# qwertyhgb/Prostate-Cancer-Multimodal-Segmentation

Hardware: AMD Instinct MI355X
Metric: train volumes/sec (5ch 128x128x64) (higher is better)
Workload: dtype bf16; 1 GPU; UNet3D 5->1, 2 x 5x128x128x64 per GPU, BCEDiceLoss, Adam(1e-4, wd 1e-5); global_batch=2, parallelism=dp1

## Files before the change

include/pcms_hip.h:

```cpp
#ifndef PCMS_HIP_H
#define PCMS_HIP_H
#include <hip/hip_runtime.h>

#ifdef __cplusplus
extern "C" {
#endif

#define PCMS_CONV_ACCUMULATE 1
#define PCMS_CONV_RELU 2
#define PCMS_GRAD_STORE 1
#define PCMS_STEM_DENSE 16

int pcms_pack_input(int dtype, const float* in, void* out, int N, int Cin, long V, int Cp, hipStream_t s);

int pcms_conv3_chunk(int dtype);
int pcms_conv3_pack_elems(int dtype, int J, int Kdim);
int pcms_conv3_mblocks(int N, int D, int H, int W);
int pcms_conv3_fwd_rows(int dtype, int N, int D, int H, int W, int c0, int c1, int Cout);
int pcms_conv3_big_min_boxes(int v);
int pcms_conv3_big_max_wgs(int v);
int pcms_conv3_small_box_mtw2(int v);
int pcms_conv3_fwd_box_vol(int v);
int pcms_conv3_pack(int dtype, const float* w, void* out, int Cout, int Cin, int flip, hipStream_t s);
int pcms_conv3_pack2(int dtype, const float* w, void* fwd, void* dgrad, int Cout, int Cin, hipStream_t s);
// ... 68 lines not shown
int pcms_bn_relu_bwd(int dtype, const void* da, const void* y, const float* scale, const float* shift,
                     const float* mean, const float* invstd, const float* gamma, float* part, float* coef,
                     float* dgamma, float* dbeta, void* dy, int C, long nvox, double* ws, hipStream_t s);
int pcms_bn_relu_bwd_finish(int dtype, const void* da, const void* y, const float* scale, const float* shift,
                            const float* mean, const float* invstd, const float* gamma, const float* part,
                            int rows, float* coef, float* dgamma, float* dbeta, void* dy, int C, long nvox,
                            double* ws, hipStream_t s);

int pcms_maxpool_fwd(int dtype, const void* a, void* p, int N, int D, int H, int W, int C, hipStream_t s);
int pcms_maxpool_bwd(int dtype, const void* a, const void* dp, void* da, int N, int D, int H, int W,
                     int C, hipStream_t s);
int pcms_bn_relu_pool(int dtype, const void* y, void* a, void* p, const float* scale, const float* shift,
                      int N, int D, int H, int W, int C, hipStream_t s);
int pcms_maxpool_bwd_bn_rows(int dtype, int N, int D, int H, int W, int C);
int pcms_maxpool_bwd_bn(int dtype, const void* y, const float* scale, const float* shift, const float* mean,
                        const float* invstd, const void* dp, void* da, float* part, int N, int D, int H, int W,
                        int C, hipStream_t s);
int pcms_maxpool_bwd_bn_sums(int dtype, const void* y, const float* scale, const float* shift, const float* mean,
                             const float* invstd, const void* dp, const void* da, float* part, int N, int D, int H,
                             int W, int C, hipStream_t s);
int pcms_maxpool_bn_apply(int dtype, const void* y, const float* scale, const float* shift, const float* mean,
                          const float* invstd, const float* coef, const void* dp, const void* da, void* dy, int N,
                          int D, int H, int W, int C, hipStream_t s);

int pcms_convt_fwd_stream(int v);
int pcms_convt_pack_elems(int dtype, int Cin, int Cout);
int pcms_convt_pack(int dtype, const float* w, void* out, int Cin, int Cout, int dgrad, hipStream_t s);
int pcms_convt_fwd(int dtype, const void* x, const void* wpack, const float* bias, void* out,
                   int N, int Din, int Hin, int Win, int Cin, int Cout, int Do, int Ho, int Wo, hipStream_t s);
int pcms_convt_fwd_ws_floats(int N, int Din, int Hin, int Win, int Cin, int Cout);
int pcms_convt_fwd_ws(int dtype, const void* x, const void* wpack, const float* bias, void* out, float* ws,
                      int N, int Din, int Hin, int Win, int Cin, int Cout, int Do, int Ho, int Wo, hipStream_t s);
int pcms_convt_dgrad(int dtype, const void* dout, const void* wpack_d, void* dx,
                     int N, int Din, int Hin, int Win, int Cin, int Cout, int Do, int Ho, int Wo, hipStream_t s);
int pcms_convt_dgrad_ws_floats(int N, int Din, int Hin, int Win, int Cin, int Cout);
int pcms_convt_dgrad_ws(int dtype, const void* dout, const void* wpack_d, void* dx, float* ws,
                        int N, int Din, int Hin, int Win, int Cin, int Cout, int Do, int Ho, int Wo, hipStream_t s);
int pcms_convt_wgrad_ws_floats(int N, int Din, int Hin, int Win, int Cin, int Cout, int target_wgs);
int pcms_convt_reduce_fused(int v);
int pcms_convt_wgrad_taps(int tt);
int pcms_convt_wgrad(int dtype, const void* x, const void* dout, float* dw, float* ws,
                     int N, int Din, int Hin, int Win, int Cin, int Cout, int Do, int Ho, int Wo,
                     int target_wgs, hipStream_t s);
int pcms_convt_wgrad_bias_ws_floats(int dtype, int N, int Din, int Hin, int Win, int Cin, int Cout, int target_wgs);
int pcms_convt_wgrad_bias(int dtype, const void* x, const void* dout, float* dw, float* db, float* ws, float* bws,
                          int N, int Din, int Hin, int Win, int Cin, int Cout, int Do, int Ho, int Wo,
// ... 131 lines not shown
```

prostate-cancer-multimodal-segmentation_amd/_lib.py:

```python
from __future__ import annotations

import ctypes
import os

import torch

LIB_PATH = os.environ.get("PCMS_LIB") or os.path.join(os.path.dirname(os.path.abspath(__file__)), "libpcms_hip.so")

F32, BF16, F32X3 = 0, 1, 2

SIGNATURES = {
    "pcms_pack_input": "ippiilis",
    "pcms_conv3_chunk": "i",
    "pcms_conv3_pack_elems": "iii",
    "pcms_conv3_mblocks": "iiii",
    "pcms_conv3_fwd_rows": "iiiiiiii",
    "pcms_conv3_big_min_boxes": "i",
    "pcms_conv3_big_max_wgs": "i",
    "pcms_conv3_fwd_box_vol": "i",
    "pcms_conv3_small_box_mtw2": "i",
    "pcms_conv3_pack": "ippiiis",
    "pcms_conv3_pack2": "ipppiis",
    "pcms_conv3_splits": "iii",
    "pcms_conv3_fwd": "ipipippppippiiiiiiis",
# ... 24 lines not shown
    "pcms_stem_wgrad": "ppppiiiiis",
    "pcms_stem_wgrad_bn": "ppppppppppiiiiis",
    "pcms_stem_dgrad_pack_elems": "i",
    "pcms_stem_dgrad_pack": "ippis",
    "pcms_stem_dgrad": "ipppiiiiis",
    "pcms_bn_relu_bwd_eval": "ipppppils",
    "pcms_head_bn_bwd_eval": "ippppppliis",
    "pcms_split_epilogue_rows": "l",
    "pcms_split_epilogue": "ipipppipilis",
    "pcms_bn_ws_doubles": "i",
    "pcms_bn_finalize": "piidpppppffppppps",
    "pcms_bn_eval_coeffs": "ppppfipps",
    "pcms_bn_fold": "ppppppfilpps",
    "pcms_bn_relu": "ippppils",
    "pcms_bn_bwd_rows": "iil",
    "pcms_bn_relu_bwd": "i" + "p" * 12 + "ilps",
    "pcms_maxpool_fwd": "ippiiiiis",
    "pcms_maxpool_bwd": "ipppiiiiis",
    "pcms_bn_relu_pool": "ipppppiiiiis",
    "pcms_maxpool_bwd_bn_rows": "iiiiii",
    "pcms_maxpool_bwd_bn": "ippppppppiiiiis",
    "pcms_maxpool_bwd_bn_sums": "ippppppppiiiiis",
    "pcms_maxpool_bn_apply": "ipppppppppiiiiis",
    "pcms_bn_relu_bwd_finish": "i" + "p" * 8 + "ippppilps",
    "pcms_convt_pack": "ippiiis",
    "pcms_convt_pack_elems": "iii",
    "pcms_convt_fwd_stream": "i",
    "pcms_convt_fwd": "ippppiiiiiiiiis",
    "pcms_convt_fwd_ws_floats": "iiiiii",
    "pcms_convt_fwd_ws": "ipppppiiiiiiiiis",
    "pcms_convt_dgrad": "ipppiiiiiiiiis",
    "pcms_convt_dgrad_ws_floats": "iiiiii",
    "pcms_convt_dgrad_ws": "ippppiiiiiiiiis",
    "pcms_convt_wgrad_ws_floats": "iiiiiii",
    "pcms_convt_wgrad_taps": "i",
    "pcms_convt_reduce_fused": "i",
    "pcms_bn_bwd_rows_cap": "i",
    "pcms_stream_grid_cap": "i",
    "pcms_convt_wgrad": "ippppiiiiiiiiiis",
    "pcms_convt_wgrad_bias_ws_floats": "iiiiiiii",
    "pcms_convt_wgrad_bias": "ippppppiiiiiiiiiis",
    "pcms_box_channel_sum_ws_floats": "iiiiii",
    "pcms_box_channel_sum": "ipppiiiiiiiiiiis",
    "pcms_head_fwd": "ippppliiifs",
    "pcms_head_bwd_ws_floats": "lii",
    "pcms_head_bwd": "ipppppppliis",
# ... 127 lines not shown
```

prostate-cancer-multimodal-segmentation_amd/csrc/ops_pool.hip:

```cpp
#include "ops_units.h"
#include "pcms_hip.h"

namespace {

template <typename T>
__global__ void maxpool_fwd_kernel(const T* a, T* p, int N, int D, int H, int W, int C) {
  constexpr int VEC = Elem<T>::kVec;
  const int Do = D / 2, Ho = H / 2, Wo = W / 2, CV = C / VEC;
  const long total = (long)N * Do * Ho * Wo * CV;
  for (long i = blockIdx.x * (long)blockDim.x + threadIdx.x; i < total; i += (long)gridDim.x * blockDim.x) {
    const uint32_t ii = (uint32_t)i;
    const int cv = ii % CV; uint32_t r = ii / CV;
    const int wo = r % Wo; r /= Wo;
    const int ho = r % Ho; r /= Ho;
    const int d_o = r % Do; const long n = r / Do;
    float m[VEC];
#pragma unroll
    for (int j = 0; j < VEC; ++j) m[j] = -INFINITY;
    for (int k = 0; k < 8; ++k) {
      const long vin = ((n * D + 2 * d_o + (k >> 2)) * H + 2 * ho + ((k >> 1) & 1)) * W + 2 * wo + (k & 1);
      float v[VEC];
      load16<T>(a + vin * C + cv * VEC, v);
#pragma unroll
      for (int j = 0; j < VEC; ++j)
// ... 19 lines not shown
#pragma unroll
    for (int j = 0; j < VEC; ++j) { m[j] = -INFINITY; arg[j] = 0; }
    long vin[8];
    for (int k = 0; k < 8; ++k) {
      vin[k] = ((n * D + 2 * d_o + (k >> 2)) * H + 2 * ho + ((k >> 1) & 1)) * W + 2 * wo + (k & 1);
      float v[VEC];
      load16<T>(a + vin[k] * C + cv * VEC, v);
#pragma unroll
      for (int j = 0; j < VEC; ++j)
        if (v[j] > m[j] || (v[j] != v[j] && m[j] == m[j])) { m[j] = v[j]; arg[j] = k; }
    }
    float g[VEC];
    load16<T>(dp + i * VEC, g);
    for (int k = 0; k < 8; ++k) {
      float o[VEC];
      load16<T>(da + vin[k] * C + cv * VEC, o);
#pragma unroll
      for (int j = 0; j < VEC; ++j) o[j] += (arg[j] == k) ? g[j] : 0.f;
      store16<T>(da + vin[k] * C + cv * VEC, o);
    }
  }
}

template <typename T, bool NT>
__global__ void __launch_bounds__(TPB) bn_relu_pool_kernel(const T* y, T* a, T* p, const float* scale,
                                                           const float* shift, int N, int D, int H, int W,
                                                           int C) {
  constexpr int VEC = Elem<T>::kVec;
  const int Dc = (D + 1) / 2, Hc = (H + 1) / 2, Wc = (W + 1) / 2, CV = C / VEC;
  const int Do = D / 2, Ho = H / 2, Wo = W / 2;
  const long total = (long)N * Dc * Hc * Wc * CV;
  const long stride = (long)gridDim.x * blockDim.x;
  long i = blockIdx.x * (long)blockDim.x + threadIdx.x;
  const int cv = (int)(i % CV);
  float sc[VEC], sh[VEC];
#pragma unroll
  for (int j = 0; j < VEC; ++j) { sc[j] = scale[cv * VEC + j]; sh[j] = shift[cv * VEC + j]; }
  for (; i < total; i += stride) {
    uint32_t r = (uint32_t)(i / CV);
    const int wc = r % Wc; r /= Wc;
    const int hc = r % Hc; r /= Hc;
    const int dc = r % Dc; const long n = r / Dc;
    float m[VEC];
#pragma unroll
    for (int j = 0; j < VEC; ++j) m[j] = -INFINITY;
    float v[8][VEC];
    long vin[8];
    bool in[8];
#pragma unroll
    for (int k = 0; k < 8; ++k) {
      const int d = 2 * dc + (k >> 2), h = 2 * hc + ((k >> 1) & 1), w = 2 * wc + (k & 1);
      in[k] = d < D && h < H && w < W;
      vin[k] = ((n * D + d) * H + h) * W + w;
#ifndef BRP_NTLOAD
#define BRP_NTLOAD 1
#endif
      if (in[k]) ld16<NT && BRP_NTLOAD>(y + vin[k] * C + cv * VEC, v[k]);
    }
#pragma unroll
    for (int k = 0; k < 8; ++k) {
      if (!in[k]) continue;
#pragma unroll
      for (int j = 0; j < VEC; ++j) v[k][j] = round_st<T>(bn_relu1(v[k][j], sc[j], sh[j]));
      st16<NT>(a + vin[k] * C + cv * VEC, v[k]);
#pragma unroll
      for (int j = 0; j < VEC; ++j)
        if (v[k][j] > m[j] || v[k][j] != v[k][j]) m[j] = v[k][j];
    }
    if (dc < Do && hc < Ho && wc < Wo) store16<T>(p + (((n * Do + dc) * Ho + hc) * Wo + wc) * C + cv * VEC, m);
  }
}

template <typename T, bool STORE = true>
__global__ void __launch_bounds__(TPB, 3) maxpool_bwd_bn_kernel(const T* y, const float* scale, const float* shift,
                                                             const float* mean, const float* invstd, const T* dp,
                                                             T* da, float* part, int N, int D, int H, int W,
                                                             int C) {
  constexpr int VEC = Elem<T>::kVec;
  __shared__ float red[TPB][VEC][2];
  const int Dc = (D + 1) / 2, Hc = (H + 1) / 2, Wc = (W + 1) / 2, CV = C / VEC;
  const int Do = D / 2, Ho = H / 2, Wo = W / 2;
  const long total = (long)N * Dc * Hc * Wc * CV;
  const long stride = (long)gridDim.x * blockDim.x;
  long i = blockIdx.x * (long)blockDim.x + threadIdx.x;
  const int cv = (int)(i % CV);
  float sc[VEC], sh[VEC], mu[VEC], is[VEC], sg[VEC], sgx[VEC];
#pragma unroll
  for (int j = 0; j < VEC; ++j) {
    const int c = cv * VEC + j;
    sc[j] = scale[c]; sh[j] = shift[c]; mu[j] = mean[c]; is[j] = invstd[c];
    sg[j] = 0.f; sgx[j] = 0.f;
  }
  auto unpack = [](const u32x4_t r, float (&o)[VEC]) {
    if constexpr (sizeof(T) == 2) {
#pragma unroll
      for (int q = 0; q < 4; ++q) { o[2 * q] = __uint_as_float(r[q] << 16); o[2 * q + 1] = __uint_as_float(r[q] & 0xffff0000u); }
    } else {
#pragma unroll
      for (int q = 0; q < 4; ++q) o[q] = __uint_as_float(r[q]);
    }
  };
  for (; i < total; i += stride) {
    uint32_t r = (uint32_t)(i / CV);
    const int wc = r % Wc; r /= Wc;
    const int hc = r % Hc; r /= Hc;
    const int dc = r % Dc; const long n = r / Dc;
    const bool whole = dc < Do && hc < Ho && wc < Wo;
    u32x4_t yr[8], dr[8], gr = {0u, 0u, 0u, 0u};
    const long v0 = ((n * D + 2 * dc) * H + 2 * hc) * W + 2 * wc;
    const bool ind = 2 * dc + 1 < D, inh = 2 * hc + 1 < H, inw = 2 * wc + 1 < W;
    auto vk = [&](int k) { return v0 + (long)(k >> 2) * H * W + ((k >> 1) & 1) * W + (k & 1); };
    auto ink = [&](int k) { return (!(k & 4) || ind) && (!(k & 2) || inh) && (!(k & 1) || inw); };
#pragma unroll
    for (int k = 0; k < 8; ++k) {
      yr[k] = (u32x4_t){0u, 0u, 0u, 0u};
      dr[k] = yr[k];
      if (ink(k)) {
        yr[k] = *reinterpret_cast<const u32x4_t*>(y + vk(k) * C + cv * VEC);
        dr[k] = *reinterpret_cast<const u32x4_t*>(da + vk(k) * C + cv * VEC);
      }
    }
    if (whole) gr = *reinterpret_cast<const u32x4_t*>(dp + (((n * Do + dc) * Ho + hc) * Wo + wc) * C + cv * VEC);
    float g[VEC], m[VEC];
    int arg[VEC];
    unpack(gr, g);
#pragma unroll
    for (int j = 0; j < VEC; ++j) { m[j] = -INFINITY; arg[j] = 0; }
    auto round2 = [](f32x2_t v) -> f32x2_t {
      if constexpr (sizeof(T) == 2) {
        const uint32_t u = pack_bf16x2(v[0], v[1]);
        return (f32x2_t){__uint_as_float(u << 16), __uint_as_float(u & 0xffff0000u)};
      } else {
        return v;
      }
    };
    auto z2of = [&](const float (&yv)[VEC], int q) {
      return __builtin_elementwise_fma((f32x2_t){yv[2 * q], yv[2 * q + 1]}, (f32x2_t){sc[2 * q], sc[2 * q + 1]},
                                       (f32x2_t){sh[2 * q], sh[2 * q + 1]});
    };
    if (whole) {
#pragma unroll
      for (int k = 0; k < 8; ++k) {
        float yv[VEC];
        unpack(yr[k], yv);
#pragma unroll
        for (int j = 0; j < VEC; ++j) {
          const float av = round_st<T>(bn_relu1(yv[j], sc[j], sh[j]));
          if (av > m[j] || (av != av && m[j] == m[j])) { m[j] = av; arg[j] = k; }
        }
      }
    }
#pragma unroll
    for (int k = 0; k < 8; ++k) {
      if (!ink(k)) continue;
      float yv[VEC], o[VEC];
      u32x4_t yk = yr[k];
      asm volatile("" : "+v"(yk));
      unpack(yk, yv);
      unpack(dr[k], o);
      if (whole) {
#pragma unroll
        for (int j = 0; j < VEC; ++j) o[j] += (arg[j] == k) ? g[j] : 0.f;
        if constexpr (STORE) store16<T>(da + vk(k) * C + cv * VEC, o);
// ... 98 lines not shown
          if (av > m[j] || (av != av && m[j] == m[j])) { m[j] = av; arg[j] = k; }
        }
      }
    }
#pragma unroll
    for (int k = 0; k < 8; ++k) {
      if (!ink(k)) continue;
      float yv[VEC], o[VEC], out[VEC];
      u32x4_t yk = yr[k];
      asm volatile("" : "+v"(yk));
      unpack(yk, yv);
      unpack(dr[k], o);
      if (whole) {
#pragma unroll
        for (int j = 0; j < VEC; ++j) o[j] = round_st<T>(o[j] + ((arg[j] == k) ? g[j] : 0.f));
      }
#pragma unroll
      for (int j = 0; j < VEC; ++j) out[j] = bn_bwd_dy(o[j], yv[j], sc[j], sh[j], mu[j], is[j], k1[j], k2[j], k3[j]);
      st16<NT>(dy + vk(k) * C + cv * VEC, out);
    }
  }
}

}

static int cell_grid(long total, int CV, int cap) {
  int g = stream_grid(total, TPB, cap);
  const int per = CV / std::__gcd(CV, TPB);
  return std::max(per, g / per * per);
}
static int pool_cells(int N, int D, int H, int W, long* cells) {
  *cells = (long)N * ((D + 1) / 2) * ((H + 1) / 2) * ((W + 1) / 2);
  return *cells * 8 >= (1L << 31) ? -7 : 0;
}
static bool pool_nt(int dtype, int N, int D, int H, int W, int C) {
  return (long)N * D * H * W * C * bytes_of(dtype) >= kNtBytesBn;
}

extern "C" {

int pcms_maxpool_fwd(int dtype, const void* a, void* p, int N, int D, int H, int W, int C, hipStream_t s) {
  if ((long)N * D * H * W * C >= (1L << 31)) return -7;
  const long total = (long)N * (D / 2) * (H / 2) * (W / 2) * (C / vec_of(dtype));
  const int grid = stream_grid(total, TPB);
  return for_storage(dtype, [&](auto t) {
    using T = decltype(t);
// ... 5 lines not shown
int pcms_maxpool_bwd(int dtype, const void* a, const void* dp, void* da, int N, int D, int H, int W, int C,
                     hipStream_t s) {
  if ((long)N * D * H * W * C >= (1L << 31)) return -7;
  const long total = (long)N * (D / 2) * (H / 2) * (W / 2) * (C / vec_of(dtype));
  const int grid = stream_grid(total, TPB);
  return for_storage(dtype, [&](auto t) {
    using T = decltype(t);
    hipLaunchKernelGGL(maxpool_bwd_kernel<T>, dim3(grid), dim3(TPB), 0, s, (const T*)a, (const T*)dp, (T*)da, N, D, H,
                       W, C);
    PCMS_CHECK_LAUNCH();
  });
}

int pcms_bn_relu_pool(int dtype, const void* y, void* a, void* p, const float* scale, const float* shift, int N,
                      int D, int H, int W, int C, hipStream_t s) {
  const int VEC = vec_of(dtype), CV = C / VEC;
  if (C % VEC) return -1;
  long cells;
  if (const int rc = pool_cells(N, D, H, W, &cells)) return rc;
  const int grid = cell_grid(cells * CV, CV, 8192);
  return for_stream(dtype, pool_nt(dtype, N, D, H, W, C), [&](auto t, auto nt) {
    using T = decltype(t);
    hipLaunchKernelGGL((bn_relu_pool_kernel<T, decltype(nt)::value>), dim3(grid), dim3(TPB), 0, s, (const T*)y, (T*)a,
                       (T*)p, scale, shift, N, D, H, W, C);
    PCMS_CHECK_LAUNCH();
  });
}

int pcms_maxpool_bwd_bn_rows(int dtype, int N, int D, int H, int W, int C) {
  const int CV = C / vec_of(dtype);
  long cells;
  pool_cells(N, D, H, W, &cells);
  return cell_grid(cells * CV, CV, g_bn_rows_cap);
}

static int maxpool_bwd_bn_any(bool store, int dtype, const void* y, const float* scale, const float* shift,
                              const float* mean, const float* invstd, const void* dp, void* da, float* part, int N,
                              int D, int H, int W, int C, hipStream_t s) {
  const int VEC = vec_of(dtype);
  if (C % VEC || TPB % (C / VEC)) return -1;
  long cells;
  if (const int rc = pool_cells(N, D, H, W, &cells)) return rc;
  const int grid = pcms_maxpool_bwd_bn_rows(dtype, N, D, H, W, C);
  return for_stream(dtype, store, [&](auto t, auto st) {
    using T = decltype(t);
    hipLaunchKernelGGL((maxpool_bwd_bn_kernel<T, decltype(st)::value>), dim3(grid), dim3(TPB), 0, s, (const T*)y, scale,
                       shift, mean, invstd, (const T*)dp, (T*)da, part, N, D, H, W, C);
    PCMS_CHECK_LAUNCH();
  });
}

int pcms_maxpool_bwd_bn(int dtype, const void* y, const float* scale, const float* shift, const float* mean,
                        const float* invstd, const void* dp, void* da, float* part, int N, int D, int H, int W,
                        int C, hipStream_t s) {
  return maxpool_bwd_bn_any(true, dtype, y, scale, shift, mean, invstd, dp, da, part, N, D, H, W, C, s);
}

int pcms_maxpool_bwd_bn_sums(int dtype, const void* y, const float* scale, const float* shift, const float* mean,
                             const float* invstd, const void* dp, const void* da, float* part, int N, int D, int H,
                             int W, int C, hipStream_t s) {
  return maxpool_bwd_bn_any(false, dtype, y, scale, shift, mean, invstd, dp, const_cast<void*>(da), part, N, D, H, W,
                            C, s);
}

int pcms_maxpool_bn_apply(int dtype, const void* y, const float* scale, const float* shift, const float* mean,
                          const float* invstd, const float* coef, const void* dp, const void* da, void* dy, int N,
                          int D, int H, int W, int C, hipStream_t s) {
  const int VEC = vec_of(dtype), CV = C / VEC;
  if (C % VEC || TPB % CV) return -1;
  long cells;
// ... 12 lines not shown
```

prostate-cancer-multimodal-segmentation_amd/engine.py:

```python
from __future__ import annotations

import contextlib
import math
import os
from typing import Dict, List, NamedTuple, Optional, Tuple

import torch

from . import _lib
from ._lib import BF16, F32, F32X3, call, query
from .dp import module_grad_ranges
from .packs import BN_EPS, WeightPacks, gaps

BN_MOMENTUM = 0.1

_DT = {"bf16": (torch.bfloat16, BF16), "fp32": (torch.float32, F32)}


class Route(NamedTuple):
    kind: str
    splits: int
    slabs: int
    slabs16: int
    rows: int
    pack16: bool


class Layout(NamedTuple):
    N: int
    D: int
    H: int
    W: int
    act_ckpt: bool
    side_min_level: int
    convt_wgrad_side: bool
    pool_bn_apply_fused: bool
    wgrad_target: int
    split_target: int
    fuse_bnin: bool
    use_b16: bool
    switches: Tuple[int, ...]
    fwd: Tuple[Route, ...] = ()
    dgrad: Tuple[Optional[Route], ...] = ()
    bnin: Tuple[bool, ...] = ()
    pool_rows: Tuple[int, ...] = ()


class ConvSpec:
    __slots__ = ("mod", "cin", "cout", "cin_store", "fwd", "dgrad", "code", "fwd16", "dgrad16", "i")

    def __init__(self, mod, cin, cout, cin_store):
        self.mod, self.cin, self.cout, self.cin_store = mod, cin, cout, cin_store
        self.i = None
        self.fwd = None
        self.dgrad = None
        self.fwd16 = None
        self.dgrad16 = None
        self.code = None

# ... 56 lines not shown
            cs.code, cs.i = self.code, i
        self.stem_fast = self.code == BF16 and self.cp == 8
        self.stem_sup = 0
        self.stem_dense = 16 if self.nmod <= 5 else 0
        self.fuse_bnin = True
        self.use_b16 = os.environ.get("PCMS_B16", "1") != "0"
        self.packs = WeightPacks(self)
        self._flat_ptrs = None
        self.bufs = None
        self.buf_key = None
        self.layout: Optional[Layout] = None
        self.epoch = 0
        self.saved_epoch = -1
        self.saved_eval_epoch = -1
        self._folded = False
        self.act_ckpt = False
        self.split_target = 512
        self.wgrad_target = 256
        self.grad_ready = None
        self.kernel_timer = None
        self.wgrad_side_min_level = 99
        self.convt_wgrad_side = False
        self.pool_bn_apply_fused = False
        self._side_stream = None
        self._side_used = False
        self.fold_bn_eval = True
        self._bn_epoch = 0
        self._store_ranges = None
        self._gstore = False
        self._flatten()
        for bn in self.bns:
            c = bn.c
            bn.scale, bn.shift, bn.mean, bn.invstd = (torch.empty(c, device=device) for _ in range(4))

    def set_fp32_conv_mode(self, mode: str, convs=None):
        if self.code == BF16:
            raise ValueError("the bf16 build has one conv arithmetic")
        code = {"x6": F32, "x3": F32X3}[mode]
        changed = [cs for cs in self.convs if convs is None or cs.i in convs]
        for cs in changed:
            cs.code = code
        self.packs.recoded(changed)
        self.buf_key = None

    def _flatten(self):
        params = list(self.model.parameters())
# ... 188 lines not shown
            rows = query("pcms_split_epilogue_rows", N * S[0] * S[1] * S[2])
        return Route(kind, splits, slabs, sp16, rows, pack16)

    def _alloc(self, key):
        L = Layout(*key)
        N, D, H, W = key[:4]
        self.bufs = self.layout = self.buf_key = None
        S = self._levels(D, H, W)
        if min(S[4]) < 1:
            raise ValueError(f"spatial size {(D, H, W)} is too small for 4 poolings")
        nv = [N * d * h * w for (d, h, w) in S]
        C = [64 * (1 << l) for l in range(5)]
        T = self.tdtype
        dev = self.device

        def act(l, c):
            return torch.empty(nv[l] * c, dtype=T, device=dev)

        b: Dict[str, object] = {"S": S, "nv": nv, "C": C}
        b["xin"] = act(0, self.cp)
        for l in range(5):
            if l > 0:
                b[f"pool{l}"] = act(l, C[l - 1])
            for k in ("y1", "a1", "y2", "x"):
                b[f"e{l}_{k}"] = act(l, C[l])
        for l in range(4):
            for k in (("u", "a2") if L.act_ckpt else ("u", "y1", "a1", "y2", "a2")):
                b[f"d{l}_{k}"] = act(l, C[l]) if (l, k) != (0, "a2") else None
        if L.act_ckpt:
            for k in ("y1", "a1", "y2"):
                b[f"ck_{k}"] = act(0, C[0])
        for l in range(5):
            b[f"gx{l}"] = act(l, C[l])
            b[f"gA{l}"] = act(l, C[l])
            b[f"gY{l}"] = act(l, C[l])
            b[f"gZ{l}"] = act(l, C[l]) if l >= L.side_min_level else b[f"gY{l}"]
            b[f"gU{l}"] = act(l, C[l])
        self.stem_sup = query("pcms_stem_supported", N, D, H, W) if self.stem_fast else 0
        b16 = L.use_b16 and self.code == BF16
        bnin = tuple(self._bnin(blk, N, S[l]) for blk, l in zip(self.enc + self.dec, (0, 1, 2, 3, 4, 3, 2, 1, 0)))
        rows_f = max(max(query("pcms_conv3_mblocks", N, *S[l]) for l in range(5)),
                     query("pcms_stem_fwd_rows", N, *S[0]))
        ws = [query("pcms_stem_wgrad_ws_floats", N, *S[0], self.nmod)] if self.stem_fast else [1]
        yacc = 1
        fwd, dgrad = [], []
        for cs, l, c0, c1 in self._sites():
# ... 79 lines not shown

    def _conv(self, cs: ConvSpec, x0, c0, x1, c1, y, N, S, stats: bool, training: bool, bn: BNSpec,
              recompute: bool = False, bnin: Optional[BNSpec] = None):
        b = self.bufs
        nvox = N * S[0] * S[1] * S[2]
        r = self.layout.fwd[cs.i]
        st = b["stats"] if training and not recompute else None
        self._launch(r, cs, cs.fwd16, cs.fwd, x0, c0, x1, c1, cs.mod.bias, y, None, cs.cout, cs.cout, st, N, S, bnin)
        if recompute:
            return
        m = bn.mod
        if training:
            if nvox <= 1:
                raise ValueError(f"Expected more than 1 value per channel when training, got input size "
                                 f"torch.Size([{N}, {bn.c}, {S[0]}, {S[1]}, {S[2]}])")
            call("pcms_bn_finalize", st, r.rows, bn.c, float(nvox), m.weight, m.bias, m.running_mean,
                 m.running_var, m.num_batches_tracked, BN_MOMENTUM, BN_EPS, bn.scale, bn.shift, bn.mean,
                 bn.invstd, b["bnws"])
        else:
            call("pcms_bn_eval_coeffs", m.weight, m.bias, m.running_mean, m.running_var, BN_EPS, bn.c,
                 bn.scale, bn.shift)

    def _block_fwd(self, blk: BlockSpec, x0, c0, x1, c1, out: Dict[str, torch.Tensor], N, S, training,
                   recompute: bool = False, pool_out=None):
        nvox = N * S[0] * S[1] * S[2]
        if not training and self._folded:
            i0 = blk.c0.i
            a2 = out["a2"] if out["a2"] is not None else out["y2"]
            self._conv_eval(i0, x0, c0, x1, c1, out["a1"], N, S)
            self._conv_eval(i0 + 1, out["a1"], blk.c0.cout, None, 0, a2, N, S)
            if pool_out is not None:
                call("pcms_maxpool_fwd", self.code, a2, pool_out, N, *S, blk.c1.cout)
            return
        self._conv(blk.c0, x0, c0, x1, c1, out["y1"], N, S, True, training, blk.b0, recompute)
        if self.layout.bnin[blk.c0.i // 2]:
            self._conv(blk.c1, out["y1"], blk.c0.cout, None, 0, out["y2"], N, S, True, training, blk.b1, recompute,
                       bnin=blk.b0)
        else:
            call("pcms_bn_relu", self.code, out["y1"], out["a1"], blk.b0.scale, blk.b0.shift, blk.c0.cout, nvox)
            self._conv(blk.c1, out["a1"], blk.c0.cout, None, 0, out["y2"], N, S, True, training, blk.b1, recompute)
        if recompute or out["a2"] is None:
            return
        if pool_out is not None:
            call("pcms_bn_relu_pool", self.code, out["y2"], out["a2"], pool_out, blk.b1.scale, blk.b1.shift, N, *S,
                 blk.c1.cout)
        else:
            call("pcms_bn_relu", self.code, out["y2"], out["a2"], blk.b1.scale, blk.b1.shift, blk.c1.cout, nvox)

    def _dec_acts(self, l: int) -> Dict[str, torch.Tensor]:
        b = self.bufs
        if not self.layout.act_ckpt:
            return {k: b[f"d{l}_{k}"] for k in ("y1", "a1", "y2", "a2")}
        n = b["nv"][l] * b["C"][l]
        return {"y1": b["ck_y1"][:n], "a1": b["ck_a1"][:n], "y2": b["ck_y2"][:n], "a2": b[f"d{l}_a2"]}

    def forward(self, x: torch.Tensor, training: bool, act: int = 0, threshold: float = 0.5,
                keep_input_grad: bool = False) -> torch.Tensor:
        if keep_input_grad and training:
            raise ValueError("keep_input_grad is the eval route; a training forward keeps its activations anyway")
        if x.dim() != 5 or x.shape[1] != self.nmod:
            raise ValueError(f"expected input (N, {self.nmod}, D, H, W), got {tuple(x.shape)}")
        if x.device != self.device:
            raise ValueError(f"input on {x.device}, model on {self.device}")
        x = x.contiguous()
        if x.dtype != torch.float32:
            x = x.float()
        N, _, D, H, W = x.shape
        key = (N, D, H, W, self.act_ckpt, self.wgrad_side_min_level, self.convt_wgrad_side, self.pool_bn_apply_fused,
               self.wgrad_target, self.split_target, self.fuse_bnin, self.use_b16, _lib.switches())
        if key != self.buf_key:
            self._alloc(key)
        self._ensure_packs()
        folded = self._folded = not training and self.fold_bn_eval and not keep_input_grad
        if folded:
            self.packs.ensure_eval()
        else:
            self._bn_epoch += training
        b = self.bufs
        S, C = b["S"], b["C"]
        call("pcms_pack_input", self.code, x, b["xin"], N, self.nmod, D * H * W, self.cp)
        inp, cin = b["xin"], self.cp
        for l in range(5):
            if l > 0:
                inp, cin = b[f"pool{l}"], C[l - 1]
            out = {"y1": b[f"e{l}_y1"], "a1": b[f"e{l}_a1"], "y2": b[f"e{l}_y2"], "a2": b[f"e{l}_x"]}
            self._block_fwd(self.enc[l], inp, cin, None, 0, out, N, S[l], training,
                            pool_out=b[f"pool{l + 1}"] if l < 4 else None)
        h = b["e4_x"]
        for i in range(4):
            l = 3 - i
            up = self.ups[i]
            fpack, _ = self.convt_packs[i]
            call("pcms_convt_fwd_ws", self.code, h, fpack, up.bias, b[f"d{l}_u"], b["ctws"], N, *S[l + 1],
                 up.in_channels, up.out_channels, *S[l])
            self._block_fwd(self.dec[i], b[f"e{l}_x"], C[l], b[f"d{l}_u"], C[l], self._dec_acts(l), N, S[l],
                            training)
            h = b[f"d{l}_a2"]
        logits = torch.empty((N, self.ncls, D, H, W), dtype=torch.float32, device=self.device)
        oc = self.model.outc
        bn = self.dec[3].b1
        if folded:
            call("pcms_head_fwd", self.code, self._dec_acts(0)["y2"], oc.weight, oc.bias, logits, D * H * W, N,
                 self.ncls, int(act), float(threshold))
        else:
            call("pcms_head_bn_fwd", self.code, self._dec_acts(0)["y2"], bn.scale, bn.shift, oc.weight, oc.bias,
                 logits, D * H * W, N, self.ncls, int(act), float(threshold))
        self.epoch += 1
        if training:
            self.saved_epoch = self.epoch
        elif keep_input_grad:
            self.saved_eval_epoch = self.epoch
        return logits

    def _stem_dgrad(self, dy1, N, S) -> torch.Tensor:
        dpack = self.packs.stem_dgrad_pack()
        dx = torch.empty((N, self.nmod, *S), dtype=torch.float32, device=self.device)
        with self._timed("stem_dgrad"):
            call("pcms_stem_dgrad", self.code, dy1, dpack, dx, N, *S, self.nmod)
        return dx

    def _block_bwd(self, blk: BlockSpec, ga2, acts, x0, c0, x1, c1, gx_out0, gx_out1, cy0, N, S, lvl,
                   bn1_rows: int = 0, pool_dp=None, want_dx: bool = False):
        b = self.bufs
        wt = self.layout.wgrad_target
        nvox = N * S[0] * S[1] * S[2]
        self._join_side()
        gY, gZ, gA = b[f"gY{lvl}"], b[f"gZ{lvl}"], b[f"gA{lvl}"]
        if ga2 is not None and bn1_rows:
            m = blk.b1.mod
            call("pcms_bn_relu_bwd_finish", self.code, ga2, acts["y2"], blk.b1.scale, blk.b1.shift, blk.b1.mean,
                 blk.b1.invstd, m.weight, b["stats"], bn1_rows, b["coef"], m.weight.grad, m.bias.grad,
                 gY if pool_dp is None else None, blk.b1.c, nvox, b["bnws"])
            if pool_dp is not None:
                call("pcms_maxpool_bn_apply", self.code, acts["y2"], blk.b1.scale, blk.b1.shift, blk.b1.mean,
                     blk.b1.invstd, b["coef"], pool_dp, ga2, gY, N, *S, blk.b1.c)
        elif ga2 is not None:
            self._bn_bwd(blk.b1, ga2, acts["y2"], gY, nvox)
        if ga2 is not None:
            self._grads_done(blk.b1.mod.weight, blk.b1.mod.bias)
        with self._side(lvl):
            if self.layout.bnin[blk.c0.i // 2]:
                call("pcms_conv3_wgrad_bnin", blk.c1.code, acts["y1"], blk.c0.cout, blk.b0.scale, blk.b0.shift, gY,
                     blk.c1.mod.weight.grad, b["dwt"], N, *S, blk.c1.cout, blk.c1.cin, wt, int(self._gstore))
            else:
                call("pcms_conv3_wgrad", blk.c1.code, acts["a1"], blk.c0.cout, None, 0, gY, blk.c1.mod.weight.grad,
                     b["dwt"], N, *S, blk.c1.cout, blk.c1.cin, wt, int(self._gstore))
        self._grads_done(blk.c1.mod.weight, blk.c1.mod.bias)
        self._dgrad(blk.c1, gY, gA, None, blk.c1.cin, N, S)
        if blk is self.enc[0] and self.stem_sup & 2:
            bn = blk.b0
            m = bn.mod
            if want_dx and gZ is gY:
                self._join_side()
            call("pcms_bn_relu_bwd", self.code, gA, acts["y1"], bn.scale, bn.shift, bn.mean, bn.invstd, m.weight,
                 b["stats"], b["coef"], m.weight.grad, m.bias.grad, gZ if want_dx else None, bn.c, nvox, b["bnws"])
            self._grads_done(m.weight, m.bias)
# ... 50 lines not shown
        g = None
        for i in reversed(range(4)):
            l = 3 - i
            blk = self.dec[i]
            acts = self._dec_acts(l)
            self._join_side()
            if L.act_ckpt:
                self._block_fwd(blk, b[f"e{l}_x"], C[l], b[f"d{l}_u"], C[l], acts, N, S[l], True, recompute=True)
            gu = b[f"gU{l}"]
            self._block_bwd(blk, g, acts, b[f"e{l}_x"], C[l], b[f"d{l}_u"], C[l], b[f"gx{l}"], gu, C[l], N,
                            S[l], l)
            up = self.ups[i]
            _, dpack = self.convt_packs[i]
            hin = b["e4_x"] if i == 0 else b[f"d{l + 1}_a2"]
            with self._side(l, L.convt_wgrad_side):
                call("pcms_convt_wgrad_bias", self.code, hin, gu, up.weight.grad, up.bias.grad,
                     b["ctws_w"] if L.convt_wgrad_side else b["ctws"], b["redws"], N, *S[l + 1], up.in_channels,
                     up.out_channels, *S[l], 512)
            self._grads_done(up.weight, up.bias)
            gnext = b["gx4"] if i == 0 else b[f"gA{l + 1}"]
            call("pcms_convt_dgrad_ws", self.code, gu, dpack, gnext, b["ctws"], N, *S[l + 1], up.in_channels,
                 up.out_channels, *S[l])
            g = gnext
        rows, pool_dp, dx = 0, None, None
        for l in reversed(range(5)):
            blk = self.enc[l]
            acts = {"y1": b[f"e{l}_y1"], "a1": b[f"e{l}_a1"], "y2": b[f"e{l}_y2"]}
            if l == 0:
                dx = self._block_bwd(blk, b["gx0"], acts, b["xin"], self.cp, None, 0, None, None, 0, N, S[0], 0,
                                     bn1_rows=rows, pool_dp=pool_dp, want_dx=want_dx)
            else:
                gp = b[f"gU{l}"]
                self._block_bwd(blk, b[f"gx{l}"], acts, b[f"pool{l}"], C[l - 1], None, 0, gp, None, C[l - 1], N,
                                S[l], l, bn1_rows=rows, pool_dp=pool_dp)
                bn = self.enc[l - 1].b1
                call("pcms_maxpool_bwd_bn_sums" if L.pool_bn_apply_fused else "pcms_maxpool_bwd_bn", self.code,
                     b[f"e{l - 1}_y2"], bn.scale, bn.shift, bn.mean, bn.invstd, gp, b[f"gx{l - 1}"], b["stats"], N,
                     *S[l - 1], C[l - 1])
                pool_dp = gp if L.pool_bn_apply_fused else None
                rows = L.pool_rows[l - 1]
        self._join_side()
        self.saved_epoch = -1
        return dx

    def _block_bwd_input(self, blk: BlockSpec, ga2, acts, gx_out0, gx_out1, cy0, N, S, lvl, stem: bool = False):
        b = self.bufs
        nvox = N * S[0] * S[1] * S[2]
        gY, gZ, gA = b[f"gY{lvl}"], b[f"gZ{lvl}"], b[f"gA{lvl}"]
        if ga2 is not None:
            call("pcms_bn_relu_bwd_eval", self.code, ga2, acts["y2"], blk.b1.scale, blk.b1.shift, gY, blk.b1.c, nvox)
        self._dgrad(blk.c1, gY, gA, None, blk.c1.cin, N, S)
        call("pcms_bn_relu_bwd_eval", self.code, gA, acts["y1"], blk.b0.scale, blk.b0.shift, gZ, blk.b0.c, nvox)
        if stem:
            return self._stem_dgrad(gZ, N, S)
        self._dgrad(blk.c0, gZ, gx_out0, gx_out1, cy0, N, S)
        return None

    def backward_input(self, dlogits: torch.Tensor) -> torch.Tensor:
        if self.saved_eval_epoch != self.epoch:
            raise RuntimeError("UNet3D input-gradient backward must follow its own eval forward (the engine "
                               "keeps only the activations of the latest forward)")
        L = self.layout
# ... 36 lines not shown
```

Baseline: 168.4 volumes/s.

## Store maxpool argmax bytes in forward to avoid recomputing pool winners in backward

The fused BN+ReLU+maxpool forward now also writes a per-element uint8 argmax index into new per-level buffers. In backward, a new sums-only kernel and a new apply kernel read that index instead of re-reading all eight inputs and redoing BN and max to find the winner, and the apply is deferred into the pooled-level BN backward. The aim is to cut backward recomputation and memory reads of the full-resolution y2 per pool window. The cost is extra forward byte writes, extra buffers, and a bf16 tie-breaking scheme that packs the window position into the comparison key.

Measured after the change: 166.8 volumes/s. Within noise of the previous version (-1.0%).

```diff
diff --git a/include/pcms_hip.h b/include/pcms_hip.h
--- a/include/pcms_hip.h
+++ b/include/pcms_hip.h
@@ -114,6 +114,14 @@
 int pcms_maxpool_bn_apply(int dtype, const void* y, const float* scale, const float* shift, const float* mean,
                           const float* invstd, const float* coef, const void* dp, const void* da, void* dy, int N,
                           int D, int H, int W, int C, hipStream_t s);
+int pcms_bn_relu_pool_arg(int dtype, const void* y, void* a, void* p, void* arg, const float* scale,
+                          const float* shift, int N, int D, int H, int W, int C, hipStream_t s);
+int pcms_maxpool_bwd_bn_sums_arg(int dtype, const void* y, const float* scale, const float* shift, const float* mean,
+                                 const float* invstd, const void* dp, const void* arg, const void* da, float* part,
+                                 int N, int D, int H, int W, int C, hipStream_t s);
+int pcms_maxpool_arg_bn_apply(int dtype, const void* y, const float* scale, const float* shift, const float* mean,
+                              const float* invstd, const float* coef, const void* dp, const void* arg,
+                              const void* da, void* dy, int N, int D, int H, int W, int C, hipStream_t s);
 
 int pcms_convt_fwd_stream(int v);
 int pcms_convt_pack_elems(int dtype, int Cin, int Cout);
diff --git a/prostate-cancer-multimodal-segmentation_amd/_lib.py b/prostate-cancer-multimodal-segmentation_amd/_lib.py
--- a/prostate-cancer-multimodal-segmentation_amd/_lib.py
+++ b/prostate-cancer-multimodal-segmentation_amd/_lib.py
@@ -70,6 +70,9 @@
     "pcms_maxpool_bwd_bn": "ippppppppiiiiis",
     "pcms_maxpool_bwd_bn_sums": "ippppppppiiiiis",
     "pcms_maxpool_bn_apply": "ipppppppppiiiiis",
+    "pcms_bn_relu_pool_arg": "ippppppiiiiis",
+    "pcms_maxpool_bwd_bn_sums_arg": "i" + "p" * 9 + "iiiiis",
+    "pcms_maxpool_arg_bn_apply": "i" + "p" * 10 + "iiiiis",
     "pcms_bn_relu_bwd_finish": "i" + "p" * 8 + "ippppilps",
     "pcms_convt_pack": "ippiiis",
     "pcms_convt_pack_elems": "iii",
diff --git a/prostate-cancer-multimodal-segmentation_amd/csrc/ops_pool.hip b/prostate-cancer-multimodal-segmentation_amd/csrc/ops_pool.hip
--- a/prostate-cancer-multimodal-segmentation_amd/csrc/ops_pool.hip
+++ b/prostate-cancer-multimodal-segmentation_amd/csrc/ops_pool.hip
@@ -65,10 +65,33 @@
   }
 }
 
-template <typename T, bool NT>
+template <int VEC>
+__device__ __forceinline__ void store_arg(uint8_t* p, const uint32_t (&k)[VEC]) {
+  const uint32_t w0 = k[0] | (k[1] << 8) | (k[2] << 16) | (k[3] << 24);
+  if constexpr (VEC == 8) {
+    const uint32_t w1 = k[4] | (k[5] << 8) | (k[6] << 16) | (k[7] << 24);
+    *reinterpret_cast<u32x2_t*>(p) = (u32x2_t){w0, w1};
+  } else {
+    *reinterpret_cast<uint32_t*>(p) = w0;
+  }
+}
+template <int VEC>
+__device__ __forceinline__ void load_arg(const uint8_t* p, uint32_t (&k)[VEC]) {
+  uint32_t w[VEC / 4];
+  if constexpr (VEC == 8) {
+    const u32x2_t v = *reinterpret_cast<const u32x2_t*>(p);
+    w[0] = v[0]; w[1] = v[1];
+  } else {
+    w[0] = *reinterpret_cast<const uint32_t*>(p);
+  }
+#pragma unroll
+  for (int j = 0; j < VEC; ++j) k[j] = (w[j / 4] >> (8 * (j % 4))) & 0xffu;
+}
+
+template <typename T, bool NT, bool ARG = false>
 __global__ void __launch_bounds__(TPB) bn_relu_pool_kernel(const T* y, T* a, T* p, const float* scale,
                                                            const float* shift, int N, int D, int H, int W,
-                                                           int C) {
+                                                           int C, uint8_t* arg = nullptr) {
   constexpr int VEC = Elem<T>::kVec;
   const int Dc = (D + 1) / 2, Hc = (H + 1) / 2, Wc = (W + 1) / 2, CV = C / VEC;
   const int Do = D / 2, Ho = H / 2, Wo = W / 2;
@@ -85,8 +108,9 @@
     const int hc = r % Hc; r /= Hc;
     const int dc = r % Dc; const long n = r / Dc;
     float m[VEC];
-#pragma unroll
-    for (int j = 0; j < VEC; ++j) m[j] = -INFINITY;
+    [[maybe_unused]] uint32_t am[VEC];
+#pragma unroll
+    for (int j = 0; j < VEC; ++j) { m[j] = -INFINITY; am[j] = 0u; }
     float v[8][VEC];
     long vin[8];
     bool in[8];
@@ -100,6 +124,39 @@
 #endif
       if (in[k]) ld16<NT && BRP_NTLOAD>(y + vin[k] * C + cv * VEC, v[k]);
     }
+    if constexpr (ARG && sizeof(T) == 2) {
+      uint32_t key[VEC];
+#pragma unroll
+      for (int j = 0; j < VEC; ++j) key[j] = 0u;
+#pragma unroll
+      for (int k = 0; k < 8; ++k) {
+        if (!in[k]) continue;
+        u32x4_t u;
+#pragma unroll
+        for (int q = 0; q < 4; ++q)
+          u[q] = pack_bf16x2(bn_relu1(v[k][2 * q], sc[2 * q], sh[2 * q]),
+                             bn_relu1(v[k][2 * q + 1], sc[2 * q + 1], sh[2 * q + 1]));
+        u32x4_t* ap = reinterpret_cast<u32x4_t*>(a + vin[k] * C + cv * VEC);
+        if constexpr (NT) __builtin_nontemporal_store(u, ap); else *ap = u;
+        const uint32_t tie = 7u - k;
+#pragma unroll
+        for (int q = 0; q < 4; ++q) {
+          key[2 * q] = max(key[2 * q], (u[q] << 16) | tie);
+          key[2 * q + 1] = max(key[2 * q + 1], (u[q] & 0xffff0000u) | tie);
+        }
+      }
+      if (dc < Do && hc < Ho && wc < Wo) {
+        const long e = (((n * Do + dc) * Ho + hc) * Wo + wc) * C + cv * VEC;
+        u32x4_t pw;
+#pragma unroll
+        for (int q = 0; q < 4; ++q) pw[q] = (key[2 * q] >> 16) | (key[2 * q + 1] & 0xffff0000u);
+        *reinterpret_cast<u32x4_t*>(p + e) = pw;
+#pragma unroll
+        for (int j = 0; j < VEC; ++j) am[j] = 7u - (key[j] & 7u);
+        store_arg<VEC>(arg + e, am);
+      }
+      continue;
+    }
 #pragma unroll
     for (int k = 0; k < 8; ++k) {
       if (!in[k]) continue;
@@ -107,18 +164,26 @@
       for (int j = 0; j < VEC; ++j) v[k][j] = round_st<T>(bn_relu1(v[k][j], sc[j], sh[j]));
       st16<NT>(a + vin[k] * C + cv * VEC, v[k]);
 #pragma unroll
-      for (int j = 0; j < VEC; ++j)
+      for (int j = 0; j < VEC; ++j) {
+        if constexpr (ARG)
+          if (v[k][j] > m[j] || (v[k][j] != v[k][j] && m[j] == m[j])) am[j] = k;
         if (v[k][j] > m[j] || v[k][j] != v[k][j]) m[j] = v[k][j];
-    }
-    if (dc < Do && hc < Ho && wc < Wo) store16<T>(p + (((n * Do + dc) * Ho + hc) * Wo + wc) * C + cv * VEC, m);
-  }
-}
-
-template <typename T, bool STORE = true>
+      }
+    }
+    if (dc < Do && hc < Ho && wc < Wo) {
+      const long e = (((n * Do + dc) * Ho + hc) * Wo + wc) * C + cv * VEC;
+      store16<T>(p + e, m);
+      if constexpr (ARG) store_arg<VEC>(arg + e, am);
+    }
+  }
+}
+
+template <typename T, bool STORE = true, bool ARG = false>
 __global__ void __launch_bounds__(TPB, 3) maxpool_bwd_bn_kernel(const T* y, const float* scale, const float* shift,
                                                              const float* mean, const float* invstd, const T* dp,
                                                              T* da, float* part, int N, int D, int H, int W,
-                                                             int C) {
+                                                             int C, const uint8_t* argp = nullptr) {
+  static_assert(!(ARG && STORE), "the argmax-byte form leaves da to maxpool_arg_bn_apply_kernel");
   constexpr int VEC = Elem<T>::kVec;
   __shared__ float red[TPB][VEC][2];
   const int Dc = (D + 1) / 2, Hc = (H + 1) / 2, Wc = (W + 1) / 2, CV = C / VEC;
@@ -164,11 +229,18 @@
       }
     }
     if (whole) gr = *reinterpret_cast<const u32x4_t*>(dp + (((n * Do + dc) * Ho + hc) * Wo + wc) * C + cv * VEC);
-    float g[VEC], m[VEC];
+    float g[VEC];
+    [[maybe_unused]] float m[VEC];
     int arg[VEC];
+    [[maybe_unused]] uint32_t ab[VEC];
+#pragma unroll
+    for (int j = 0; j < VEC; ++j) { m[j] = -INFINITY; arg[j] = 0; ab[j] = 0u; }
+    if constexpr (ARG) {
+      if (whole) load_arg<VEC>(argp + (((n * Do + dc) * Ho + hc) * Wo + wc) * C + cv * VEC, ab);
+#pragma unroll
+      for (int j = 0; j < VEC; ++j) arg[j] = (int)ab[j];
+    }
     unpack(gr, g);
-#pragma unroll
-    for (int j = 0; j < VEC; ++j) { m[j] = -INFINITY; arg[j] = 0; }
     auto round2 = [](f32x2_t v) -> f32x2_t {
       if constexpr (sizeof(T) == 2) {
         const uint32_t u = pack_bf16x2(v[0], v[1]);
@@ -181,7 +253,7 @@
       return __builtin_elementwise_fma((f32x2_t){yv[2 * q], yv[2 * q + 1]}, (f32x2_t){sc[2 * q], sc[2 * q + 1]},
                                        (f32x2_t){sh[2 * q], sh[2 * q + 1]});
     };
-    if (whole) {
+    if (!ARG && whole) {
 #pragma unroll
       for (int k = 0; k < 8; ++k) {
         float yv[VEC];
@@ -326,6 +398,81 @@
   }
 }
 
+template <typename T, bool NT>
+__global__ void __launch_bounds__(TPB) maxpool_arg_bn_apply_kernel(
+    const T* y, const float* scale, const float* shift, const float* mean, const float* invstd, const float* coef,
+    const T* dp, const uint8_t* argp, const T* gx, T* dy, int N, int D, int H, int W, int C) {
+  constexpr int VEC = Elem<T>::kVec;
+  const int CG = C / VEC;
+  const int cg = threadIdx.x % CG, vl = threadIdx.x / CG, VL = TPB / CG;
+  const int c0 = cg * VEC;
+  float sc[VEC], sh[VEC], mu[VEC], is[VEC], k1[VEC], k2[VEC], k3[VEC];
+#pragma unroll
+  for (int j = 0; j < VEC; ++j) {
+    const int c = c0 + j;
+    sc[j] = scale[c]; sh[j] = shift[c]; mu[j] = mean[c]; is[j] = invstd[c];
+    k1[j] = coef[c * 3]; k2[j] = coef[c * 3 + 1]; k3[j] = coef[c * 3 + 2];
+  }
+  const int Wp = (W + 1) / 2, Do = D / 2, Ho = H / 2, Wo = W / 2;
+  const uint32_t pairs = (uint32_t)N * D * H * Wp;
+  for (uint32_t p = blockIdx.x * VL + vl; p < pairs; p += gridDim.x * VL) {
+    const uint32_t row = p / Wp;
+    const int wp = (int)(p - row * Wp);
+    uint32_t r = row;
+    const int h = r % H; r /= H;
+    const int d = r % D; const long n = r / D;
+    const long v = (long)row * W + 2 * wp;
+    const bool two = 2 * wp + 1 < W;
+    const bool whole = (d >> 1) < Do && (h >> 1) < Ho && wp < Wo;
+    auto ldraw = [](const T* q) -> u32x4_t {
+      if constexpr (NT) return __builtin_nontemporal_load(reinterpret_cast<const u32x4_t*>(q));
+      else return *reinterpret_cast<const u32x4_t*>(q);
+    };
+    auto unpack = [](const u32x4_t w, float (&o)[VEC]) {
+      if constexpr (sizeof(T) == 2) {
+#pragma unroll
+        for (int q = 0; q < 4; ++q) { o[2 * q] = __uint_as_float(w[q] << 16); o[2 * q + 1] = __uint_as_float(w[q] & 0xffff0000u); }
+      } else {
+#pragma unroll
+        for (int q = 0; q < 4; ++q) o[q] = __uint_as_float(w[q]);
+      }
+    };
+    const u32x4_t zero = {0u, 0u, 0u, 0u};
+    u32x4_t yr[2] = {zero, zero}, gr[2] = {zero, zero}, pr = zero;
+    uint32_t am[VEC];
+#pragma unroll
+    for (int j = 0; j < VEC; ++j) am[j] = 0u;
+    yr[0] = ldraw(y + v * C + c0);
+    gr[0] = ldraw(gx + v * C + c0);
+    if (two) {
+      yr[1] = ldraw(y + (v + 1) * C + c0);
+      gr[1] = ldraw(gx + (v + 1) * C + c0);
+    }
+    if (whole) {
+      const long e = (((n * Do + (d >> 1)) * Ho + (h >> 1)) * Wo + wp) * C + c0;
+      pr = *reinterpret_cast<const u32x4_t*>(dp + e);
+      load_arg<VEC>(argp + e, am);
+    }
+    float gp[VEC];
+    unpack(pr, gp);
+    const uint32_t ka = ((d & 1) << 2) | ((h & 1) << 1);
+#pragma unroll
+    for (int t = 0; t < 2; ++t) {
+      if (t == 1 && !two) break;
+      float yv[VEC], g[VEC], o[VEC];
+      unpack(yr[t], yv);
+      unpack(gr[t], g);
+      if (whole) {
+#pragma unroll
+        for (int j = 0; j < VEC; ++j) g[j] = round_st<T>(g[j] + ((am[j] == ka + t) ? gp[j] : 0.f));
+      }
+#pragma unroll
+      for (int j = 0; j < VEC; ++j) o[j] = bn_bwd_dy(g[j], yv[j], sc[j], sh[j], mu[j], is[j], k1[j], k2[j], k3[j]);
+      st16<NT>(dy + (v + t) * C + c0, o);
+    }
+  }
+}
+
 }
 
 static int cell_grid(long total, int CV, int cap) {
@@ -377,7 +524,23 @@
   return for_stream(dtype, pool_nt(dtype, N, D, H, W, C), [&](auto t, auto nt) {
     using T = decltype(t);
     hipLaunchKernelGGL((bn_relu_pool_kernel<T, decltype(nt)::value>), dim3(grid), dim3(TPB), 0, s, (const T*)y, (T*)a,
-                       (T*)p, scale, shift, N, D, H, W, C);
+                       (T*)p, scale, shift, N, D, H, W, C, (uint8_t*)nullptr);
+    PCMS_CHECK_LAUNCH();
+  });
+}
+
+int pcms_bn_relu_pool_arg(int dtype, const void* y, void* a, void* p, void* arg, const float* scale,
+                          const float* shift, int N, int D, int H, int W, int C, hipStream_t s) {
+  const int VEC = vec_of(dtype), CV = C / VEC;
+  if (C % VEC) return -1;
+  if (!arg || misaligned(arg, 8)) return -2;
+  long cells;
+  if (const int rc = pool_cells(N, D, H, W, &cells)) return rc;
+  const int grid = cell_grid(cells * CV, CV, 8192);
+  return for_stream(dtype, pool_nt(dtype, N, D, H, W, C), [&](auto t, auto nt) {
+    using T = decltype(t);
+    hipLaunchKernelGGL((bn_relu_pool_kernel<T, decltype(nt)::value, true>), dim3(grid), dim3(TPB), 0, s, (const T*)y,
+                       (T*)a, (T*)p, scale, shift, N, D, H, W, C, (uint8_t*)arg);
     PCMS_CHECK_LAUNCH();
   });
 }
@@ -400,7 +563,44 @@
   return for_stream(dtype, store, [&](auto t, auto st) {
     using T = decltype(t);
     hipLaunchKernelGGL((maxpool_bwd_bn_kernel<T, decltype(st)::value>), dim3(grid), dim3(TPB), 0, s, (const T*)y, scale,
-                       shift, mean, invstd, (const T*)dp, (T*)da, part, N, D, H, W, C);
+                       shift, mean, invstd, (const T*)dp, (T*)da, part, N, D, H, W, C, (const uint8_t*)nullptr);
+    PCMS_CHECK_LAUNCH();
+  });
+}
+
+int pcms_maxpool_bwd_bn_sums_arg(int dtype, const void* y, const float* scale, const float* shift, const float* mean,
+                                 const float* invstd, const void* dp, const void* arg, const void* da, float* part,
+                                 int N, int D, int H, int W, int C, hipStream_t s) {
+  const int VEC = vec_of(dtype);
+  if (C % VEC || TPB % (C / VEC)) return -1;
+  if (!arg || misaligned(arg, 8)) return -2;
+  long cells;
+  if (const int rc = pool_cells(N, D, H, W, &cells)) return rc;
+  const int grid = pcms_maxpool_bwd_bn_rows(dtype, N, D, H, W, C);
+  return for_storage(dtype, [&](auto t) {
+    using T = decltype(t);
+    hipLaunchKernelGGL((maxpool_bwd_bn_kernel<T, false, true>), dim3(grid), dim3(TPB), 0, s, (const T*)y, scale, shift,
+                       mean, invstd, (const T*)dp, (T*)const_cast<void*>(da), part, N, D, H, W, C,
+                       (const uint8_t*)arg);
+    PCMS_CHECK_LAUNCH();
+  });
+}
+
+int pcms_maxpool_arg_bn_apply(int dtype, const void* y, const float* scale, const float* shift, const float* mean,
+                              const float* invstd, const float* coef, const void* dp, const void* arg,
+                              const void* da, void* dy, int N, int D, int H, int W, int C, hipStream_t s) {
+  const int VEC = vec_of(dtype);
+  if (C % VEC || TPB % (C / VEC)) return -1;
+  if (!arg || misaligned(arg, 8)) return -2;
+  long cells;
+  if (const int rc = pool_cells(N, D, H, W, &cells)) return rc;
+  const int VL = TPB / (C / VEC);
+  const int grid = stream_grid((long)N * D * H * ((W + 1) / 2), VL, 8192);
+  return for_stream(dtype, pool_nt(dtype, N, D, H, W, C), [&](auto t, auto nt) {
+    using T = decltype(t);
+    hipLaunchKernelGGL((maxpool_arg_bn_apply_kernel<T, decltype(nt)::value>), dim3(grid), dim3(TPB), 0, s, (const T*)y,
+                       scale, shift, mean, invstd, coef, (const T*)dp, (const uint8_t*)arg, (const T*)da, (T*)dy, N, D,
+                       H, W, C);
     PCMS_CHECK_LAUNCH();
   });
 }
diff --git a/prostate-cancer-multimodal-segmentation_amd/engine.py b/prostate-cancer-multimodal-segmentation_amd/engine.py
--- a/prostate-cancer-multimodal-segmentation_amd/engine.py
+++ b/prostate-cancer-multimodal-segmentation_amd/engine.py
@@ -35,6 +35,7 @@
     side_min_level: int
     convt_wgrad_side: bool
     pool_bn_apply_fused: bool
+    pool_argmax: bool
     wgrad_target: int
     split_target: int
     fuse_bnin: bool
@@ -137,6 +138,7 @@
         self.wgrad_side_min_level = 99
         self.convt_wgrad_side = False
         self.pool_bn_apply_fused = False
+        self.pool_argmax = True
         self._side_stream = None
         self._side_used = False
         self.fold_bn_eval = True
@@ -371,6 +373,8 @@
         for l in range(5):
             if l > 0:
                 b[f"pool{l}"] = act(l, C[l - 1])
+                if L.pool_argmax and not L.pool_bn_apply_fused:
+                    b[f"parg{l}"] = torch.empty(nv[l] * C[l - 1], dtype=torch.uint8, device=dev)
             for k in ("y1", "a1", "y2", "x"):
                 b[f"e{l}_{k}"] = act(l, C[l])
         for l in range(4):
@@ -496,7 +500,7 @@
                  bn.scale, bn.shift)
 
     def _block_fwd(self, blk: BlockSpec, x0, c0, x1, c1, out: Dict[str, torch.Tensor], N, S, training,
-                   recompute: bool = False, pool_out=None):
+                   recompute: bool = False, pool_out=None, pool_arg=None):
         nvox = N * S[0] * S[1] * S[2]
         if not training and self._folded:
             i0 = blk.c0.i
@@ -515,7 +519,10 @@
             self._conv(blk.c1, out["a1"], blk.c0.cout, None, 0, out["y2"], N, S, True, training, blk.b1, recompute)
         if recompute or out["a2"] is None:
             return
-        if pool_out is not None:
+        if pool_arg is not None:
+            call("pcms_bn_relu_pool_arg", self.code, out["y2"], out["a2"], pool_out, pool_arg, blk.b1.scale,
+                 blk.b1.shift, N, *S, blk.c1.cout)
+        elif pool_out is not None:
             call("pcms_bn_relu_pool", self.code, out["y2"], out["a2"], pool_out, blk.b1.scale, blk.b1.shift, N, *S,
                  blk.c1.cout)
         else:
@@ -541,7 +548,7 @@
             x = x.float()
         N, _, D, H, W = x.shape
         key = (N, D, H, W, self.act_ckpt, self.wgrad_side_min_level, self.convt_wgrad_side, self.pool_bn_apply_fused,
-               self.wgrad_target, self.split_target, self.fuse_bnin, self.use_b16, _lib.switches())
+               self.pool_argmax, self.wgrad_target, self.split_target, self.fuse_bnin, self.use_b16, _lib.switches())
         if key != self.buf_key:
             self._alloc(key)
         self._ensure_packs()
@@ -559,7 +566,8 @@
                 inp, cin = b[f"pool{l}"], C[l - 1]
             out = {"y1": b[f"e{l}_y1"], "a1": b[f"e{l}_a1"], "y2": b[f"e{l}_y2"], "a2": b[f"e{l}_x"]}
             self._block_fwd(self.enc[l], inp, cin, None, 0, out, N, S[l], training,
-                            pool_out=b[f"pool{l + 1}"] if l < 4 else None)
+                            pool_out=b[f"pool{l + 1}"] if l < 4 else None,
+                            pool_arg=b.get(f"parg{l + 1}") if training else None)
         h = b["e4_x"]
         for i in range(4):
             l = 3 - i
@@ -594,7 +602,7 @@
         return dx
 
     def _block_bwd(self, blk: BlockSpec, ga2, acts, x0, c0, x1, c1, gx_out0, gx_out1, cy0, N, S, lvl,
-                   bn1_rows: int = 0, pool_dp=None, want_dx: bool = False):
+                   bn1_rows: int = 0, pool_dp=None, pool_arg=None, want_dx: bool = False):
         b = self.bufs
         wt = self.layout.wgrad_target
         nvox = N * S[0] * S[1] * S[2]
@@ -605,7 +613,10 @@
             call("pcms_bn_relu_bwd_finish", self.code, ga2, acts["y2"], blk.b1.scale, blk.b1.shift, blk.b1.mean,
                  blk.b1.invstd, m.weight, b["stats"], bn1_rows, b["coef"], m.weight.grad, m.bias.grad,
                  gY if pool_dp is None else None, blk.b1.c, nvox, b["bnws"])
-            if pool_dp is not None:
+            if pool_arg is not None:
+                call("pcms_maxpool_arg_bn_apply", self.code, acts["y2"], blk.b1.scale, blk.b1.shift, blk.b1.mean,
+                     blk.b1.invstd, b["coef"], pool_dp, pool_arg, ga2, gY, N, *S, blk.b1.c)
+            elif pool_dp is not None:
                 call("pcms_maxpool_bn_apply", self.code, acts["y2"], blk.b1.scale, blk.b1.shift, blk.b1.mean,
                      blk.b1.invstd, b["coef"], pool_dp, ga2, gY, N, *S, blk.b1.c)
         elif ga2 is not None:
@@ -702,22 +713,27 @@
             call("pcms_convt_dgrad_ws", self.code, gu, dpack, gnext, b["ctws"], N, *S[l + 1], up.in_channels,
                  up.out_channels, *S[l])
             g = gnext
-        rows, pool_dp, dx = 0, None, None
+        rows, pool_dp, pool_arg, dx = 0, None, None, None
         for l in reversed(range(5)):
             blk = self.enc[l]
             acts = {"y1": b[f"e{l}_y1"], "a1": b[f"e{l}_a1"], "y2": b[f"e{l}_y2"]}
             if l == 0:
                 dx = self._block_bwd(blk, b["gx0"], acts, b["xin"], self.cp, None, 0, None, None, 0, N, S[0], 0,
-                                     bn1_rows=rows, pool_dp=pool_dp, want_dx=want_dx)
+                                     bn1_rows=rows, pool_dp=pool_dp, pool_arg=pool_arg, want_dx=want_dx)
             else:
                 gp = b[f"gU{l}"]
                 self._block_bwd(blk, b[f"gx{l}"], acts, b[f"pool{l}"], C[l - 1], None, 0, gp, None, C[l - 1], N,
-                                S[l], l, bn1_rows=rows, pool_dp=pool_dp)
+                                S[l], l, bn1_rows=rows, pool_dp=pool_dp, pool_arg=pool_arg)
                 bn = self.enc[l - 1].b1
-                call("pcms_maxpool_bwd_bn_sums" if L.pool_bn_apply_fused else "pcms_maxpool_bwd_bn", self.code,
-                     b[f"e{l - 1}_y2"], bn.scale, bn.shift, bn.mean, bn.invstd, gp, b[f"gx{l - 1}"], b["stats"], N,
-                     *S[l - 1], C[l - 1])
-                pool_dp = gp if L.pool_bn_apply_fused else None
+                pool_arg = b.get(f"parg{l}")
+                if pool_arg is not None:
+                    call("pcms_maxpool_bwd_bn_sums_arg", self.code, b[f"e{l - 1}_y2"], bn.scale, bn.shift, bn.mean,
+                         bn.invstd, gp, pool_arg, b[f"gx{l - 1}"], b["stats"], N, *S[l - 1], C[l - 1])
+                else:
+                    call("pcms_maxpool_bwd_bn_sums" if L.pool_bn_apply_fused else "pcms_maxpool_bwd_bn", self.code,
+                         b[f"e{l - 1}_y2"], bn.scale, bn.shift, bn.mean, bn.invstd, gp, b[f"gx{l - 1}"], b["stats"],
+                         N, *S[l - 1], C[l - 1])
+                pool_dp = gp if L.pool_bn_apply_fused or pool_arg is not None else None
                 rows = L.pool_rows[l - 1]
         self._join_side()
         self.saved_epoch = -1
```
